# joesound212985/Deepfake-Detection-using-CLIP-Based-SigLIP-2-Vision-Transformers

Hardware: AMD Instinct MI355X
Metric: images/sec (train fwd+bwd) SigLIP-2-so400m@384 bf16 (higher is better)
Workload: dtype bf16; 1 GPU; so400m-patch14-384 encoder+pool-head train fwd+bwd, 384x384, per-GPU batch 128, seeded random weights; global_batch=128, parallelism=dp1

## Files before the change

deepfake-detection-using-clip-based-siglip-2-vision-transformers_amd/csrc/attention.hip:

```cpp
#include <stdlib.h>

#include "common.hip.h"
#include "kernels.h"

namespace sgl {

hipError_t attn_f32_fwd(const float*, const float*, const float*, float*, float*, int, int, int, int, int, int, hipStream_t);
hipError_t attn_f32_bwd(const float*, const float*, const float*, const float*, const float*, const float*, float*,
                        float*, int, int, int, int, int, int, hipStream_t);
hipError_t attn_ref_fwd(const float*, const float*, const float*, float*, float*, int, int, int, int, int, int, hipStream_t);
hipError_t attn_ref_bwd(const float*, const float*, const float*, const float*, const float*, const float*, float*,
                        float*, int, int, int, int, int, int, hipStream_t);

template <int DP>
struct AttnCfg {
  static constexpr int KS = DP / 16;
  static constexpr int DT = (DP + 31) / 32;
  static constexpr int CPR = DP / 8;
  static constexpr int RSTR = DP * 2 + 16;
  static constexpr int TSTR = 192;
  static constexpr int DSTR = 208;
};

__device__ __forceinline__ u32x4 a_ldg(__amdgpu_buffer_rsrc_t r, uint32_t off) {
  return __builtin_amdgcn_raw_buffer_load_b128(r, off, 0, 0);
}
template <typename T>
__device__ __forceinline__ lo_x8<T> as_x8(u32x4 v) { return __builtin_bit_cast(lo_x8<T>, v); }
template <typename T>
__device__ __forceinline__ lo_x8<T> lds_row8(const char* p) { return *reinterpret_cast<const lo_x8<T>*>(p); }
template <typename T>
__device__ __forceinline__ lo_x4<T> lds_tr4(const char* p) { return lds_read_tr16<T>(p); }
template <typename T>
__device__ __forceinline__ lo_x8<T> lds_trfrag(const char* img, int stride, int kk, int dcol0, int lane) {
  const int g = lane >> 4, q = (lane >> 2) & 3, p = lane & 3;
  const char* a = img + (16 * kk + 4 * (g >> 1) + q) * stride + (dcol0 + 16 * (g & 1) + 4 * p) * 2;
  const lo_x4<T> lo = lds_tr4<T>(a);
  const lo_x4<T> hi = lds_tr4<T>(a + 8 * stride);
  return __builtin_shufflevector(lo, hi, 0, 1, 2, 3, 4, 5, 6, 7);
}
template <typename T>
__device__ __forceinline__ lo_x8<T> pack8(const f32x16& s, int base) {
  lo_x8<T> r;
#pragma unroll
  for (int j = 0; j < 8; ++j) r[j] = (T)s[base + j];
  return r;
}
__device__ __forceinline__ float fast_exp2(float x) { return __builtin_amdgcn_exp2f(x); }

__device__ __forceinline__ bool head_block(int nb, int BH, int& bh, int& xb) {
  const int pid = blockIdx.x, xcd = pid & 7, slot = pid >> 3;
  const int hq = slot / nb;
  bh = hq * 8 + xcd;
  xb = slot - hq * nb;
  return bh < BH;
}
static inline dim3 head_grid(int nb, int BH) { return dim3((unsigned)(8 * ((BH + 7) / 8) * nb)); }

struct HeadSrc {
  uint32_t rowbytes, nc, bytes;
  size_t base;
};
__device__ __forceinline__ HeadSrc head_src(int ld, int b, int hd, int H, int N, int dh, int DP) {
  HeadSrc r;
  if (ld > 0) {
    r.rowbytes = (uint32_t)ld * 2u;
    r.nc = (uint32_t)dh / 8u;
    r.bytes = (uint32_t)(((size_t)(N - 1) * ld + dh) * 2);
    r.base = (size_t)b * N * ld + (size_t)hd * dh;
  } else {
    r.rowbytes = (uint32_t)DP * 2u;
    r.nc = (uint32_t)DP / 8u;
    r.bytes = (uint32_t)((size_t)N * DP * 2);
    r.base = ((size_t)b * H + hd) * (size_t)N * DP;
  }
  return r;
}

#define MFMA32(a, b, c) mfma_32x32x16((a), (b), (c))

__device__ __forceinline__ void att_dma16(u32x4 desc, uint32_t lds_addr, uint32_t voff) {
  asm volatile("s_mov_b32 m0, %0\n\ts_nop 0\n\tbuffer_load_dwordx4 %1, %2, 0 offen lds" ::"s"(lds_addr), "v"(voff), "s"(desc)
               : "memory");
}
__device__ __forceinline__ void att_dma4(u32x4 desc, uint32_t lds_addr, uint32_t voff) {
  asm volatile("s_mov_b32 m0, %0\n\ts_nop 0\n\tbuffer_load_dword %1, %2, 0 offen lds" ::"s"(lds_addr), "v"(voff), "s"(desc)
               : "memory");
}
__device__ __forceinline__ u32x4 att_desc(const void* base, uint32_t bytes) {
  const uint64_t q = (uint64_t)base;
  return u32x4{(uint32_t)q, (uint32_t)(q >> 32) & 0xffffu, bytes, 0x00020000u};
}
__device__ __forceinline__ uint32_t att_chunk_off(int cidx, int rows, int SC, int NC, uint32_t rowbytes) {
  const int row = cidx / SC, col = cidx - row * SC;
  return (row < rows && col < NC) ? (uint32_t)row * rowbytes + (uint32_t)col * 16u : SGL_OOB;
}
#define SGL_ATT_WAIT_BARRIER(n)                                   \
  do {                                                            \
    asm volatile("s_waitcnt vmcnt(" #n ") lgkmcnt(0)" ::: "memory"); \
    __builtin_amdgcn_sched_barrier(0);                            \
    __builtin_amdgcn_s_barrier();                                 \
    __builtin_amdgcn_sched_barrier(0);                            \
    asm volatile("" ::: "memory");                                \
  } while (0)

template <typename T, int DP, bool TOK>
__global__ __launch_bounds__(256) __attribute__((amdgpu_waves_per_eu(3, 3))) void attn_fwd_kernel(const T* __restrict__ Q, const T* __restrict__ K,
                                                          const T* __restrict__ V, T* __restrict__ out,
                                                          float* __restrict__ lse, int B, int H, int N, int dh, int ld,
                                                          float c, float scale) {
  using C = AttnCfg<DP>;
  constexpr int KT = 64;
  constexpr int KBYTES = KT * C::RSTR, VBYTES = KT * C::TSTR, STAGE = KBYTES + VBYTES;
  constexpr int SCK = C::RSTR / 16, SCV = C::TSTR / 16;
  constexpr int NIK = KT * SCK / 64, NIV = KT * SCV / 64, NSLOT = NIK + NIV;
  constexpr int NPW = (NSLOT + 3) / 4;
  static_assert(KT * SCK % 64 == 0 && KT * SCV % 64 == 0, "whole DMA instructions per image");
  extern __shared__ __attribute__((aligned(16))) char smem[];
  const int t = threadIdx.x, lane = t & 63;
  const int w = __builtin_amdgcn_readfirstlane(t >> 6);
  int bh, xb;
  if (!head_block((N + 127) / 128, B * H, bh, xb)) return;
  const int b = bh / H, hd = bh - b * H;
  const int q0 = xb * 128 + w * 32;
  HeadSrc src = head_src(TOK ? ld : 0, b, hd, H, N, dh, DP);
  if constexpr (!TOK) {
    src.rowbytes = (uint32_t)DP * 2u;
    src.nc = (uint32_t)DP / 8u;
  }
  const __amdgpu_buffer_rsrc_t rq = make_rsrc(Q + src.base, src.bytes);
  const u32x4 dk_ = att_desc(K + src.base, src.bytes);
  const u32x4 dv_ = att_desc(V + src.base, src.bytes);
  const uint32_t lds0 = (uint32_t)(size_t)((SGL_LDS char*)smem);

  const int qi = lane & 31, hh = lane >> 5;
  lo_x8<T> qf[C::KS];
#pragma unroll
  for (int ks = 0; ks < C::KS; ++ks) {
    const uint32_t ch = (uint32_t)(2 * ks + hh);
    qf[ks] = as_x8<T>(a_ldg(rq, (q0 + qi < N && ch < src.nc) ? (uint32_t)(q0 + qi) * src.rowbytes + ch * 16u : SGL_OOB));
  }

  uint32_t voff[NPW];
#pragma unroll
  for (int j = 0; j < NPW; ++j) {
    const int sl = w + 4 * j;
    voff[j] = (sl < NIK) ? att_chunk_off(sl * 64 + lane, KT, SCK, (int)src.nc, src.rowbytes)
                         : att_chunk_off((sl - NIK) * 64 + lane, KT, SCV, (int)src.nc, src.rowbytes);
  }
  const uint32_t tile_adv = (uint32_t)KT * src.rowbytes;
  auto issue = [&](int stage) {
    const uint32_t sb = lds0 + (uint32_t)(stage * STAGE);
#pragma unroll
    for (int j = 0; j < NPW; ++j) {
      const int sl = w + 4 * j;
      if (sl < NSLOT) att_dma16(sl < NIK ? dk_ : dv_, sb + (uint32_t)sl * 1024u, voff[j]);
      voff[j] += tile_adv;
    }
  };

  float m_run = -INFINITY, l_run = 0.f;
  f32x16 o[C::DT];
#pragma unroll
  for (int dt = 0; dt < C::DT; ++dt)
#pragma unroll
    for (int r = 0; r < 16; ++r) o[dt][r] = 0.f;

  const int ntiles = (N + KT - 1) / KT;
#pragma unroll
  for (int ks = 0; ks < C::KS; ++ks) asm volatile("" ::"v"(qf[ks]));
  asm volatile("s_waitcnt vmcnt(0)" ::: "memory");
  issue(0);
  for (int tile = 0; tile < ntiles; ++tile) {
    const int cur = tile & 1;
    SGL_ATT_WAIT_BARRIER(0);
    if (tile + 1 < ntiles) issue(cur ^ 1);
    const char* kb = smem + cur * STAGE;
    const char* vb = kb + KBYTES;
    f32x16 s0, s1;
#pragma unroll
    for (int r = 0; r < 16; ++r) { s0[r] = 0.f; s1[r] = 0.f; }
#pragma unroll
    for (int ks = 0; ks < C::KS; ++ks) {
      const lo_x8<T> k0 = lds_row8<T>(kb + qi * C::RSTR + (16 * ks + 8 * hh) * 2);
      const lo_x8<T> k1 = lds_row8<T>(kb + (qi + 32) * C::RSTR + (16 * ks + 8 * hh) * 2);
      s0 = MFMA32(k0, qf[ks], s0);
      s1 = MFMA32(k1, qf[ks], s1);
    }
    if (tile == ntiles - 1) {
#pragma unroll
      for (int r = 0; r < 16; ++r) {
        const int key = tile * KT + (r & 3) + 8 * (r >> 2) + 4 * hh;
        if (key >= N) s0[r] = -INFINITY;
        if (key + 32 >= N) s1[r] = -INFINITY;
      }
    }
    float mx = s0[0];
#pragma unroll
    for (int r = 1; r < 16; ++r) mx = fmaxf(mx, s0[r]);
#pragma unroll
    for (int r = 0; r < 16; ++r) mx = fmaxf(mx, s1[r]);
    mx = fmaxf(mx, __shfl_xor(mx, 32, 64));
    const float m_new = fmaxf(m_run, mx);
    const bool grew = __any(m_new > m_run);
    const float alpha = grew ? fast_exp2(c * (m_run - m_new)) : 1.0f;
    const float mc = m_new * c;
    float rs = 0.f;
#pragma unroll
    for (int r = 0; r < 16; ++r) {
      s0[r] = fast_exp2(fmaf(s0[r], c, -mc));
      s1[r] = fast_exp2(fmaf(s1[r], c, -mc));
      rs += s0[r] + s1[r];
    }
    l_run = l_run * alpha + rs;
    m_run = m_new;
    if (grew) {
#pragma unroll
      for (int dt = 0; dt < C::DT; ++dt)
#pragma unroll
        for (int r = 0; r < 16; ++r) o[dt][r] *= alpha;
    }
    lo_x8<T> pb[4];
    pb[0] = pack8<T>(s0, 0);
    pb[1] = pack8<T>(s0, 8);
    pb[2] = pack8<T>(s1, 0);
    pb[3] = pack8<T>(s1, 8);
#pragma unroll
    for (int dt = 0; dt < C::DT; ++dt)
#pragma unroll
      for (int kk = 0; kk < 4; ++kk) o[dt] = MFMA32(lds_trfrag<T>(vb, C::TSTR, kk, dt * 32, lane), pb[kk], o[dt]);
  }
  const float l = l_run + __shfl_xor(l_run, 32, 64);
  const float inv = 1.0f / l;
  const int q = q0 + qi;
  if (q < N) {
    T* orow = out + ((size_t)b * N + q) * ((size_t)H * dh) + hd * dh;
#pragma unroll
    for (int dt = 0; dt < C::DT; ++dt)
#pragma unroll
      for (int g4 = 0; g4 < 4; ++g4) {
        const int d = dt * 32 + 8 * g4 + 4 * hh;
        if (d < dh) {
          lo_x4<T> v4;
#pragma unroll
          for (int r = 0; r < 4; ++r) v4[r] = (T)(o[dt][4 * g4 + r] * inv);
          *reinterpret_cast<lo_x4<T>*>(orow + d) = v4;
        }
      }
    if (hh == 0) lse[(size_t)bh * N + q] = m_run * scale + __logf(l);
  }
}

template <typename T, int DP, bool TOK>
__global__ __launch_bounds__(256, 2) void attn_bwd_kv_kernel(const T* __restrict__ Q, const T* __restrict__ K,
                                                             const T* __restrict__ V, const T* __restrict__ dO,
                                                             const float* __restrict__ aux, T* __restrict__ dqkv,
                                                             int B, int H, int N, int dh, int ld, float c, float scale) {
  using C = AttnCfg<DP>;
  constexpr int QT = 32;
  constexpr int SC = C::DSTR / 16;
  constexpr int NIS = (QT * SC + 63) / 64;
  constexpr int IMG = NIS * 1024;
  constexpr int STAGE = 2 * IMG + QT * 8;
  constexpr int NSLOT = 2 * NIS + 1;
  static_assert(NSLOT <= 16 && NSLOT > 12, "four DMA slots per wave (three for the last wave)");
  extern __shared__ __attribute__((aligned(16))) char smem[];
  const int t = threadIdx.x, lane = t & 63;
  const int w = __builtin_amdgcn_readfirstlane(t >> 6);
  int bh, xb;
  if (!head_block((N + 127) / 128, B * H, bh, xb)) return;
  const int b = bh / H, hd = bh - b * H;
  const int D = H * dh;
  const int key0 = xb * 128 + w * 32;
  HeadSrc src = head_src(TOK ? ld : 0, b, hd, H, N, dh, DP);
  if constexpr (!TOK) {
    src.rowbytes = (uint32_t)DP * 2u;
    src.nc = (uint32_t)DP / 8u;
  }
  const __amdgpu_buffer_rsrc_t rk = make_rsrc(K + src.base, src.bytes);
  const __amdgpu_buffer_rsrc_t rv = make_rsrc(V + src.base, src.bytes);
  const T* dOb = dO + (size_t)b * N * D + hd * dh;
  const u32x4 dq_ = att_desc(Q + src.base, src.bytes);
  const u32x4 ddo = att_desc(dOb, (uint32_t)(((size_t)(N - 1) * D + dh) * 2));
  const u32x4 dax = att_desc(aux + (size_t)bh * N * 2, (uint32_t)((size_t)N * 8));
  const uint32_t lds0 = (uint32_t)(size_t)((SGL_LDS char*)smem);

  const int li = lane & 31, hh = lane >> 5;
  lo_x8<T> kfr[C::KS], vfr[C::KS];
#pragma unroll
  for (int ks = 0; ks < C::KS; ++ks) {
    const uint32_t ch = (uint32_t)(2 * ks + hh);
    const uint32_t off = (key0 + li < N && ch < src.nc) ? (uint32_t)(key0 + li) * src.rowbytes + ch * 16u : SGL_OOB;
    kfr[ks] = as_x8<T>(a_ldg(rk, off));
    vfr[ks] = as_x8<T>(a_ldg(rv, off));
  }

  uint32_t voff[4], vadv[4];
  u32x4 dsc[3];
#pragma unroll
  for (int j = 0; j < 4; ++j) {
    const int sl = w + 4 * j;
    if (sl < NIS) {
      voff[j] = att_chunk_off(sl * 64 + lane, QT, SC, (int)src.nc, src.rowbytes);
      vadv[j] = (uint32_t)QT * src.rowbytes;
    } else if (sl < 2 * NIS) {
      voff[j] = att_chunk_off((sl - NIS) * 64 + lane, QT, SC, dh / 8, (uint32_t)D * 2u);
      vadv[j] = (uint32_t)(QT * D * 2);
    } else {
      voff[j] = (uint32_t)lane * 4u;
      vadv[j] = (uint32_t)(QT * 8);
    }
    if (j < 3) dsc[j] = (sl < NIS) ? dq_ : ddo;
  }
  auto issue1 = [&](int j, int stage) {
    const uint32_t sb = lds0 + (uint32_t)(stage * STAGE) + (uint32_t)w * 1024u;
    if (j < 3) {
      att_dma16(dsc[j], sb + (uint32_t)j * 4096u, voff[j]);
    } else {
      if (w < 2) att_dma16(ddo, sb + 3u * 4096u, voff[3]);
      else if (w == 2) att_dma4(dax, lds0 + (uint32_t)(stage * STAGE + 2 * IMG), voff[3]);
    }
    voff[j] += vadv[j];
  };
  auto issue = [&](int stage) {
#pragma unroll
    for (int j = 0; j < 4; ++j) issue1(j, stage);
  };

  f32x16 dk[C::DT], dv[C::DT];
#pragma unroll
  for (int dt = 0; dt < C::DT; ++dt)
#pragma unroll
    for (int r = 0; r < 16; ++r) { dk[dt][r] = 0.f; dv[dt][r] = 0.f; }

  const int ntiles = (N + QT - 1) / QT;
#pragma unroll
  for (int ks = 0; ks < C::KS; ++ks) asm volatile("" ::"v"(kfr[ks]), "v"(vfr[ks]));
  asm volatile("s_waitcnt vmcnt(0)" ::: "memory");
  issue(0);
  issue(1);
  int st = 0;
  for (int qt = 0; qt < ntiles; ++qt) {
    if (w == 3) SGL_ATT_WAIT_BARRIER(3); else SGL_ATT_WAIT_BARRIER(4);
    const int st_next = (st == 0) ? 2 : st - 1;
    const char* qimg = smem + st * STAGE;
    const char* dimg = qimg + IMG;
    const float* ld = reinterpret_cast<const float*>(qimg + 2 * IMG);
    st = (st == 2) ? 0 : st + 1;
    f32x16 S, dP;
#pragma unroll
    for (int r = 0; r < 16; ++r) { S[r] = 0.f; dP[r] = 0.f; }
    lo_x8<T> qa[C::KS], da[C::KS];
#pragma unroll
    for (int ks = 0; ks < C::KS; ++ks) {
      qa[ks] = lds_row8<T>(qimg + li * C::DSTR + (16 * ks + 8 * hh) * 2);
      da[ks] = lds_row8<T>(dimg + li * C::DSTR + (16 * ks + 8 * hh) * 2);
    }
#pragma unroll
    for (int ks = 0; ks < C::KS; ++ks) {
      S = MFMA32(qa[ks], kfr[ks], S);
      dP = MFMA32(da[ks], vfr[ks], dP);
    }
    if constexpr (C::KS == 5) {
      __builtin_amdgcn_sched_group_barrier(0x100, 4, 0);
#pragma unroll
      for (int i = 0; i < 6; ++i) {
        __builtin_amdgcn_sched_group_barrier(0x008, 1, 0);
        __builtin_amdgcn_sched_group_barrier(0x100, 1, 0);
      }
      __builtin_amdgcn_sched_group_barrier(0x008, 4, 0);
    }
    __builtin_amdgcn_sched_barrier(0);
    constexpr int NF = 2 * 2 * C::DT;
    lo_x8<T> fr[NF];
    auto frag = [&](int i) {
      const int which = i & 1, kk = (i >> 1) & 1, dt = i >> 2;
      return lds_trfrag<T>(which ? qimg : dimg, C::DSTR, kk, dt * 32, lane);
    };
    constexpr int PRE = NF < 2 ? NF : 2;
#pragma unroll
    for (int i = 0; i < PRE; ++i) fr[i] = frag(i);
    __builtin_amdgcn_sched_barrier(0);
#pragma unroll
    for (int g4 = 0; g4 < 4; ++g4) {
      const f32x4 A0 = *reinterpret_cast<const f32x4*>(ld + 2 * (8 * g4 + 4 * hh));
      const f32x4 A1 = *reinterpret_cast<const f32x4*>(ld + 2 * (8 * g4 + 4 * hh) + 4);
      const float L4[4] = {A0[0], A0[2], A1[0], A1[2]};
      const float D4[4] = {A0[1], A0[3], A1[1], A1[3]};
#pragma unroll
      for (int r3 = 0; r3 < 4; ++r3) {
        const int r = 4 * g4 + r3;
        const float p = fast_exp2(fmaf(S[r], c, L4[r3]));
        S[r] = p;
        dP[r] = p * fmaf(dP[r], scale, D4[r3]);
      }
    }
    lo_x8<T> pb[2], dsb[2];
    pb[0] = pack8<T>(S, 0);
    pb[1] = pack8<T>(S, 8);
    dsb[0] = pack8<T>(dP, 0);
    dsb[1] = pack8<T>(dP, 8);
    __builtin_amdgcn_sched_barrier(0);
#pragma unroll
    for (int i = 0; i < NF; ++i) {
      if (i + PRE < NF) fr[i + PRE] = frag(i + PRE);
      const int which = i & 1, kk = (i >> 1) & 1, dt = i >> 2;
      if (which) dk[dt] = MFMA32(fr[i], dsb[kk], dk[dt]);
      else dv[dt] = MFMA32(fr[i], pb[kk], dv[dt]);
      if (i % 3 == 1) issue1(i / 3, st_next);
      __builtin_amdgcn_sched_barrier(0);
    }
#pragma unroll
    for (int j = (NF + 1) / 3; j < 4; ++j) issue1(j, st_next);
  }
  asm volatile("s_waitcnt vmcnt(0)" ::: "memory");
  const int key = key0 + li;
  if (key < N) {
    T* krow = dqkv + ((size_t)b * N + key) * (3 * (size_t)D) + D + hd * dh;
    T* vrow = krow + D;
#pragma unroll
    for (int dt = 0; dt < C::DT; ++dt)
#pragma unroll
      for (int g4 = 0; g4 < 4; ++g4) {
        const int d = dt * 32 + 8 * g4 + 4 * hh;
        if (d < dh) {
          lo_x4<T> a, g;
#pragma unroll
          for (int r = 0; r < 4; ++r) {
            a[r] = (T)dk[dt][4 * g4 + r];
            g[r] = (T)dv[dt][4 * g4 + r];
          }
          *reinterpret_cast<lo_x4<T>*>(krow + d) = a;
          *reinterpret_cast<lo_x4<T>*>(vrow + d) = g;
        }
      }
  }
}

template <typename T, int DP, bool TOK>
__global__ __launch_bounds__(256, 2) void attn_bwd_q_kernel(const T* __restrict__ Q, const T* __restrict__ K,
                                                            const T* __restrict__ V, const T* __restrict__ O,
                                                            const T* __restrict__ dO, const float* __restrict__ lse,
                                                            float* __restrict__ aux, T* __restrict__ dqkv,
                                                            int B, int H, int N, int dh, int ld, float c, float scale) {
  using C = AttnCfg<DP>;
  constexpr int KT = 32;
  constexpr int SCK = C::DSTR / 16, SCV = C::RSTR / 16;
  constexpr int NIK = (KT * SCK + 63) / 64, NIV = (KT * SCV + 63) / 64;
  constexpr int KIMG = NIK * 1024, VIMG = NIV * 1024, STAGE = KIMG + VIMG;
  constexpr int NSLOT = NIK + NIV;
  static_assert(NSLOT <= 16, "at most four DMA slots per wave");
  constexpr float LOG2E = 1.4426950408889634f;
  extern __shared__ __attribute__((aligned(16))) char smem[];
  const int t = threadIdx.x, lane = t & 63;
  const int w = __builtin_amdgcn_readfirstlane(t >> 6);
  int bh, xb;
  if (!head_block((N + 127) / 128, B * H, bh, xb)) return;
  const int b = bh / H, hd = bh - b * H;
  const int D = H * dh;
  const int q0 = xb * 128 + w * 32;
  HeadSrc src = head_src(TOK ? ld : 0, b, hd, H, N, dh, DP);
  if constexpr (!TOK) {
    src.rowbytes = (uint32_t)DP * 2u;
    src.nc = (uint32_t)DP / 8u;
  }
  const __amdgpu_buffer_rsrc_t rq = make_rsrc(Q + src.base, src.bytes);
  const T* dOb = dO + (size_t)b * N * D + hd * dh;
  const __amdgpu_buffer_rsrc_t rdo = make_rsrc(dOb, (uint32_t)(((size_t)(N - 1) * D + dh) * 2));
  const u32x4 dk_ = att_desc(K + src.base, src.bytes);
  const u32x4 dv_ = att_desc(V + src.base, src.bytes);
  const uint32_t lds0 = (uint32_t)(size_t)((SGL_LDS char*)smem);

  const int li = lane & 31, hh = lane >> 5;
  const int q = q0 + li;
  lo_x8<T> qf[C::KS], dof[C::KS];
#pragma unroll
  for (int ks = 0; ks < C::KS; ++ks) {
    const int col = 16 * ks + 8 * hh;
    qf[ks] = as_x8<T>(a_ldg(rq, (q < N && (uint32_t)(col >> 3) < src.nc) ? (uint32_t)q * src.rowbytes + (uint32_t)col * 2u
                                                                           : SGL_OOB));
    dof[ks] = as_x8<T>(a_ldg(rdo, (q < N && col < dh) ? (uint32_t)(((size_t)q * D + col) * 2) : SGL_OOB));
  }
  float dl = 0.f;
  {
    const __amdgpu_buffer_rsrc_t ro = make_rsrc(O + (size_t)b * N * D + hd * dh, (uint32_t)(((size_t)(N - 1) * D + dh) * 2));
#pragma unroll
    for (int ks = 0; ks < C::KS; ++ks) {
      const int col = 16 * ks + 8 * hh;
      const lo_x8<T> of = as_x8<T>(a_ldg(ro, (q < N && col < dh) ? (uint32_t)(((size_t)q * D + col) * 2) : SGL_OOB));
#pragma unroll
      for (int j = 0; j < 8; ++j) dl = fmaf((float)of[j], (float)dof[ks][j], dl);
    }
    dl += __shfl_xor(dl, 32, 64);
  }
  const float Lq = (q < N) ? -lse[(size_t)bh * N + q] * LOG2E : -INFINITY;
  const float Dq = (q < N) ? -dl * scale : 0.f;
  if (q < N && hh == 0) *reinterpret_cast<float2*>(aux + 2 * ((size_t)bh * N + q)) = make_float2(Lq, Dq);

  uint32_t voff[4];
  u32x4 dsc[4];
  uint32_t ldst[4];
#pragma unroll
  for (int j = 0; j < 4; ++j) {
    const int sl = w + 4 * j;
    if (sl < NIK) {
      voff[j] = att_chunk_off(sl * 64 + lane, KT, SCK, (int)src.nc, src.rowbytes);
      dsc[j] = dk_;
      ldst[j] = (uint32_t)sl * 1024u;
    } else {
      voff[j] = att_chunk_off((sl - NIK) * 64 + lane, KT, SCV, (int)src.nc, src.rowbytes);
      dsc[j] = dv_;
      ldst[j] = (uint32_t)(KIMG + (sl - NIK) * 1024);
    }
  }
  auto issue1 = [&](int j, int stage) {
    if (w + 4 * j < NSLOT) att_dma16(dsc[j], lds0 + (uint32_t)(stage * STAGE) + ldst[j], voff[j]);
    voff[j] += (uint32_t)KT * src.rowbytes;
  };

  f32x16 dq[C::DT];
#pragma unroll
  for (int dt = 0; dt < C::DT; ++dt)
#pragma unroll
    for (int r = 0; r < 16; ++r) dq[dt][r] = 0.f;

  const int ntiles = (N + KT - 1) / KT;
#pragma unroll
  for (int ks = 0; ks < C::KS; ++ks) asm volatile("" ::"v"(qf[ks]), "v"(dof[ks]));
  asm volatile("" ::"v"(Lq), "v"(Dq));
  asm volatile("s_waitcnt vmcnt(0)" ::: "memory");
#pragma unroll
  for (int j = 0; j < 4; ++j) issue1(j, 0);
#pragma unroll
  for (int j = 0; j < 4; ++j) issue1(j, 1);
  int st = 0;
  for (int kt = 0; kt < ntiles; ++kt) {
    const int nw = (NSLOT - w + 3) / 4;
    if (nw >= 4) SGL_ATT_WAIT_BARRIER(4);
    else if (nw == 3) SGL_ATT_WAIT_BARRIER(3);
    else if (nw == 2) SGL_ATT_WAIT_BARRIER(2);
    else SGL_ATT_WAIT_BARRIER(1);
    const int st_next = (st == 0) ? 2 : st - 1;
    const char* kimg = smem + st * STAGE;
    const char* vimg = kimg + KIMG;
    st = (st == 2) ? 0 : st + 1;
    f32x16 S, dP;
#pragma unroll
    for (int r = 0; r < 16; ++r) { S[r] = 0.f; dP[r] = 0.f; }
    lo_x8<T> ka[C::KS], va[C::KS];
#pragma unroll
    for (int ks = 0; ks < C::KS; ++ks) {
      ka[ks] = lds_row8<T>(kimg + li * C::DSTR + (16 * ks + 8 * hh) * 2);
      va[ks] = lds_row8<T>(vimg + li * C::RSTR + (16 * ks + 8 * hh) * 2);
    }
#pragma unroll
    for (int ks = 0; ks < C::KS; ++ks) {
      S = MFMA32(ka[ks], qf[ks], S);
      dP = MFMA32(va[ks], dof[ks], dP);
    }
    if constexpr (C::KS == 5) {
      __builtin_amdgcn_sched_group_barrier(0x100, 6, 0);
#pragma unroll
      for (int i = 0; i < 4; ++i) {
        __builtin_amdgcn_sched_group_barrier(0x008, 1, 0);
        __builtin_amdgcn_sched_group_barrier(0x100, 1, 0);
      }
      __builtin_amdgcn_sched_group_barrier(0x008, 6, 0);
    }
    __builtin_amdgcn_sched_barrier(0);
    lo_x8<T> kt_frag[C::DT][2];
#pragma unroll
    for (int dt = 0; dt < C::DT; ++dt)
#pragma unroll
      for (int kk = 0; kk < 2; ++kk) kt_frag[dt][kk] = lds_trfrag<T>(kimg, C::DSTR, kk, dt * 32, lane);
    __builtin_amdgcn_sched_barrier(0);
#pragma unroll
    for (int r = 0; r < 16; ++r) {
      const float p = fast_exp2(fmaf(S[r], c, Lq));
      dP[r] = p * fmaf(dP[r], scale, Dq);
    }
    if (kt == ntiles - 1) {
#pragma unroll
      for (int r = 0; r < 16; ++r) {
        const int key = kt * KT + (r & 3) + 8 * (r >> 2) + 4 * hh;
        if (key >= N) dP[r] = 0.f;
      }
    }
    lo_x8<T> dsb[2];
    dsb[0] = pack8<T>(dP, 0);
    dsb[1] = pack8<T>(dP, 8);
#pragma unroll
    for (int i = 0; i < 2 * C::DT; ++i) {
      dq[i >> 1] = MFMA32(kt_frag[i >> 1][i & 1], dsb[i & 1], dq[i >> 1]);
      if (i < 4) issue1(i, st_next);
      __builtin_amdgcn_sched_barrier(0);
    }
#pragma unroll
    for (int j = 2 * C::DT; j < 4; ++j) issue1(j, st_next);
  }
  asm volatile("s_waitcnt vmcnt(0)" ::: "memory");
  if (q < N) {
    T* qrow = dqkv + ((size_t)b * N + q) * (3 * (size_t)D) + hd * dh;
#pragma unroll
    for (int dt = 0; dt < C::DT; ++dt)
#pragma unroll
      for (int g4 = 0; g4 < 4; ++g4) {
        const int d = dt * 32 + 8 * g4 + 4 * hh;
        if (d < dh) {
          lo_x4<T> a;
#pragma unroll
          for (int r = 0; r < 4; ++r) a[r] = (T)dq[dt][4 * g4 + r];
          *reinterpret_cast<lo_x4<T>*>(qrow + d) = a;
        }
      }
  }
}

template <typename T, int DP>
static hipError_t fwd_launch(const T* q, const T* k, const T* v, T* out, float* lse, int B, int H, int N,
                             int dh, int ld, hipStream_t s) {
  using C = AttnCfg<DP>;
  constexpr int smem = 2 * (64 * C::RSTR + 64 * C::TSTR);
  const float scale = 1.0f / sqrtf((float)dh);
  if (ld > 0)
    hipLaunchKernelGGL((attn_fwd_kernel<T, DP, true>), head_grid((N + 127) / 128, B * H), dim3(256), smem, s, q, k, v, out, lse,
                       B, H, N, dh, ld, scale * 1.4426950408889634f, scale);
  else
    hipLaunchKernelGGL((attn_fwd_kernel<T, DP, false>), head_grid((N + 127) / 128, B * H), dim3(256), smem, s, q, k, v, out,
                       lse, B, H, N, dh, 0, scale * 1.4426950408889634f, scale);
  return hipGetLastError();
}

template <typename T, int DP>
static hipError_t bwd_launch(const T* q, const T* k, const T* v, const T* out, const T* dout,
                             const float* lse, T* dqkv, float* delta, int B, int H, int N, int dh, int ld,
                             hipStream_t s) {
  using C = AttnCfg<DP>;
  const float scale = 1.0f / sqrtf((float)dh);
  const float c = scale * 1.4426950408889634f;
  constexpr int smem_kv = 3 * (2 * ((32 * (C::DSTR / 16) + 63) / 64) * 1024 + 32 * 8);
  constexpr int smem_q = 3 * (((32 * (C::DSTR / 16) + 63) / 64) + ((32 * (C::RSTR / 16) + 63) / 64)) * 1024;
  const dim3 grid = head_grid((N + 127) / 128, B * H), block(256);
  if (ld > 0)
    hipLaunchKernelGGL((attn_bwd_q_kernel<T, DP, true>), grid, block, smem_q, s, q, k, v, out, dout, lse, delta, dqkv, B, H, N,
                       dh, ld, c, scale);
  else
    hipLaunchKernelGGL((attn_bwd_q_kernel<T, DP, false>), grid, block, smem_q, s, q, k, v, out, dout, lse, delta, dqkv, B, H, N,
                       dh, 0, c, scale);
  hipError_t e = hipGetLastError();
  if (e != hipSuccess) return e;
  if (ld > 0)
    hipLaunchKernelGGL((attn_bwd_kv_kernel<T, DP, true>), grid, block, smem_kv, s, q, k, v, dout, delta, dqkv, B, H, N, dh, ld, c,
                       scale);
  else
    hipLaunchKernelGGL((attn_bwd_kv_kernel<T, DP, false>), grid, block, smem_kv, s, q, k, v, dout, delta, dqkv, B, H, N, dh, 0,
                       c, scale);
  return hipGetLastError();
}

static bool attn_shape_ok(int N, int dh, int DP, int H, int ld) {
  if (dh % 8 || DP != ((dh + 15) / 16) * 16) return false;
  if (DP != 16 && DP != 32 && DP != 48 && DP != 64 && DP != 80 && DP != 96) return false;
  if (ld < 0 || (ld > 0 && (ld % 8 || ld < H * dh))) return false;
  if ((size_t)N * (ld > 0 ? ld : DP) * 2 >= (1ull << 31)) return false;
  if ((size_t)N * H * dh * 2 >= (1ull << 31)) return false;
  return true;
}

hipError_t attn_fwd(const void* q, const void* k, const void* v, int dtype, void* out, float* lse, int B, int H, int N,
                    int dh, int DP, int ld, hipStream_t s) {
  if (B * H == 0 || N == 0) return hipSuccess;
  if (dtype == DT_F32)
    return attn_ref_fwd((const float*)q, (const float*)k, (const float*)v, (float*)out, lse, B, H, N, dh, DP, ld, s);
  if (dtype == DT_F32_MFMA)
    return attn_f32_fwd((const float*)q, (const float*)k, (const float*)v, (float*)out, lse, B, H, N, dh, DP, ld, s);
  if (!attn_shape_ok(N, dh, DP, H, ld)) return hipErrorInvalidValue;
  if ((((uintptr_t)q) | ((uintptr_t)k) | ((uintptr_t)v)) & 15) return hipErrorInvalidValue;
#define SGL_F(T, DPV) \
  case DPV: return fwd_launch<T, DPV>((const T*)q, (const T*)k, (const T*)v, (T*)out, lse, B, H, N, dh, ld, s);
  if (dtype == DT_F16) {
    switch (DP) {
      SGL_F(f16, 16) SGL_F(f16, 32) SGL_F(f16, 48) SGL_F(f16, 64) SGL_F(f16, 80) SGL_F(f16, 96)
    }
    return hipErrorInvalidValue;
  }
  switch (DP) {
    SGL_F(bf16, 16) SGL_F(bf16, 32) SGL_F(bf16, 48) SGL_F(bf16, 64) SGL_F(bf16, 80) SGL_F(bf16, 96)
  }
#undef SGL_F
  return hipErrorInvalidValue;
}

hipError_t attn_bwd(const void* q, const void* k, const void* v, const void* out, const void* dout, const float* lse,
                    int dtype, void* dqkv, float* delta, float* , int B, int H, int N, int dh, int DP,
                    int ld, hipStream_t s) {
  if (B * H == 0 || N == 0) return hipSuccess;
  if (dtype == DT_F32)
    return attn_ref_bwd((const float*)q, (const float*)k, (const float*)v, (const float*)out, (const float*)dout, lse,
                        (float*)dqkv, delta, B, H, N, dh, DP, ld, s);
  if (dtype == DT_F32_MFMA)
    return attn_f32_bwd((const float*)q, (const float*)k, (const float*)v, (const float*)out, (const float*)dout, lse,
                        (float*)dqkv, delta, B, H, N, dh, DP, ld, s);
  if (!attn_shape_ok(N, dh, DP, H, ld)) return hipErrorInvalidValue;
  if ((((uintptr_t)q) | ((uintptr_t)k) | ((uintptr_t)v)) & 15) return hipErrorInvalidValue;
#define SGL_B(T, DPV)                                                                                  \
  case DPV:                                                                                            \
    return bwd_launch<T, DPV>((const T*)q, (const T*)k, (const T*)v, (const T*)out, (const T*)dout, lse, \
                              (T*)dqkv, delta, B, H, N, dh, ld, s);
  if (dtype == DT_F16) {
    switch (DP) {
      SGL_B(f16, 16) SGL_B(f16, 32) SGL_B(f16, 48) SGL_B(f16, 64) SGL_B(f16, 80) SGL_B(f16, 96)
    }
    return hipErrorInvalidValue;
  }
  switch (DP) {
    SGL_B(bf16, 16) SGL_B(bf16, 32) SGL_B(bf16, 48) SGL_B(bf16, 64) SGL_B(bf16, 80) SGL_B(bf16, 96)
  }
#undef SGL_B
  return hipErrorInvalidValue;
}

}
```

Measured before the change: 439.5 images/sec.

## Use rotated swizzled LDS images in attention backward with precomputed lane bases

Replaces the padded 208-byte-stride LDS tiles for Q/dO/K in both backward kernels with a dense 192-byte rotated-chunk layout. Compile-time checks assert that row and transposed reads are bank-conflict-free. Per-lane LDS base addresses are computed once and pinned, and the 3-stage loop is unrolled so stage offsets become immediates, cutting address arithmetic. The smaller image drops one DMA slot per tile and shrinks LDS, in exchange for a more complex addressing scheme and larger unrolled code.

Result: no change. 440.6 images/sec (median of 3 runs) (+0.2%).

```diff
diff --git a/deepfake-detection-using-clip-based-siglip-2-vision-transformers_amd/csrc/attention.hip b/deepfake-detection-using-clip-based-siglip-2-vision-transformers_amd/csrc/attention.hip
--- a/deepfake-detection-using-clip-based-siglip-2-vision-transformers_amd/csrc/attention.hip
+++ b/deepfake-detection-using-clip-based-siglip-2-vision-transformers_amd/csrc/attention.hip
@@ -19,7 +19,6 @@
   static constexpr int CPR = DP / 8;
   static constexpr int RSTR = DP * 2 + 16;
   static constexpr int TSTR = 192;
-  static constexpr int DSTR = 208;
 };
 
 __device__ __forceinline__ u32x4 a_ldg(__amdgpu_buffer_rsrc_t r, uint32_t off) {
@@ -95,6 +94,127 @@
   const int row = cidx / SC, col = cidx - row * SC;
   return (row < rows && col < NC) ? (uint32_t)row * rowbytes + (uint32_t)col * 16u : SGL_OOB;
 }
+
+namespace att_img {
+constexpr int ROWS = 32, NCH = 12, ROWB = NCH * 16, BYTES = ROWS * ROWB, NDMA = BYTES / 1024;
+static_assert(BYTES % 1024 == 0, "whole DMA instructions per image");
+__host__ __device__ constexpr int slot_of(int row, int chunk) { return (chunk + (row >> 2)) % NCH; }
+__host__ __device__ constexpr int chunk_of(int row, int slot) { return (slot + NCH - (row >> 2)) % NCH; }
+__host__ __device__ constexpr int off(int row, int colb) { return row * ROWB + 16 * slot_of(row, colb >> 4) + (colb & 15); }
+
+__host__ __device__ constexpr int row_off(int lane, int ks) { return off(lane & 31, 32 * ks + 16 * (lane >> 5)); }
+
+__host__ __device__ constexpr int tr_row(int lane) { return 4 * (lane >> 5) + ((lane >> 2) & 3); }
+__host__ __device__ constexpr int tr_colb(int lane) { return 32 * ((lane >> 4) & 1) + 8 * (lane & 3); }
+__host__ __device__ constexpr int tr_off(int lane, int kk, int dt, int half) {
+  return off(16 * kk + 8 * half + tr_row(lane), 64 * dt + tr_colb(lane));
+}
+__host__ __device__ constexpr int tr_B(int kk, int dt, int half) { return (4 * (dt + kk) + 2 * half) % NCH; }
+__host__ __device__ constexpr int tr_sel(int kk, int dt, int half) { return tr_B(kk, dt, half) < 8 ? 0 : tr_B(kk, dt, half) == 8 ? 1 : 2; }
+__host__ __device__ constexpr int tr_base(int lane, int sel) {
+  return sel == 0 ? tr_off(lane, 0, 0, 0) : sel == 1 ? tr_off(lane, 0, 2, 0) : tr_off(lane, 0, 2, 1) - 8 * ROWB;
+}
+__host__ __device__ constexpr bool tr_uses(int DT, int sel) {
+  for (int kk = 0; kk < 2; ++kk)
+    for (int dt = 0; dt < DT; ++dt)
+      for (int half = 0; half < 2; ++half)
+        if (tr_sel(kk, dt, half) == sel) return true;
+  return false;
+}
+__host__ __device__ constexpr int tr_imm(int kk, int dt, int half) {
+  return (16 * kk + 8 * half) * ROWB + (tr_B(kk, dt, half) < 8 ? 16 * tr_B(kk, dt, half) : 0);
+}
+
+constexpr int b128_group(int lane) {
+  const int l = lane & 31;
+  return ((l < 4 || (l >= 12 && l < 16) || (l >= 20 && l < 28)) ? 0 : 1) + 2 * (lane >> 5);
+}
+constexpr int b64_group(int lane) { return lane >> 5; }
+template <typename Addr, typename Group>
+constexpr int lds_cycles(Addr addr, Group group, int ngroups, int dwords) {
+  int total = 0;
+  for (int g = 0; g < ngroups; ++g) {
+    int seen[64 * 4] = {}, nseen = 0, load[64] = {}, worst = 0;
+    for (int lane = 0; lane < 64; ++lane) {
+      if (group(lane) != g) continue;
+      for (int d = 0; d < dwords; ++d) {
+        const int dw = addr(lane) / 4 + d;
+        bool dup = false;
+        for (int i = 0; i < nseen; ++i) dup = dup || seen[i] == dw;
+        if (dup) continue;
+        seen[nseen++] = dw;
+        if (++load[dw % 64] > worst) worst = load[dw % 64];
+      }
+    }
+    total += worst;
+  }
+  return total;
+}
+struct RowAddr { int ks; constexpr int operator()(int lane) const { return row_off(lane, ks); } };
+struct TrAddr { int kk, dt, half; constexpr int operator()(int lane) const { return tr_base(lane, tr_sel(kk, dt, half)) + tr_imm(kk, dt, half); } };
+struct G128 { constexpr int operator()(int lane) const { return b128_group(lane); } };
+struct G64 { constexpr int operator()(int lane) const { return b64_group(lane); } };
+constexpr bool check_inverse() {
+  for (int r = 0; r < ROWS; ++r)
+    for (int c = 0; c < NCH; ++c)
+      if (chunk_of(r, slot_of(r, c)) != c || off(r, 16 * c) < 0 || off(r, 16 * c) + 16 > BYTES) return false;
+  return true;
+}
+constexpr bool check_tr_bases() {
+  for (int lane = 0; lane < 64; ++lane)
+    for (int kk = 0; kk < 2; ++kk)
+      for (int dt = 0; dt < 3; ++dt)
+        for (int half = 0; half < 2; ++half)
+          if (TrAddr{kk, dt, half}(lane) != tr_off(lane, kk, dt, half)) return false;
+  return true;
+}
+constexpr int row_read_cycles() {
+  int n = 0;
+  for (int ks = 0; ks < 6; ++ks) n += lds_cycles(RowAddr{ks}, G128{}, 4, 4);
+  return n;
+}
+constexpr int tr_read_cycles() {
+  int n = 0;
+  for (int kk = 0; kk < 2; ++kk)
+    for (int dt = 0; dt < 3; ++dt)
+      for (int half = 0; half < 2; ++half) n += lds_cycles(TrAddr{kk, dt, half}, G64{}, 2, 2);
+  return n;
+}
+static_assert(check_inverse(), "slot_of / chunk_of are inverse permutations inside the image");
+static_assert(check_tr_bases(), "three per-lane bases + immediates reproduce every transposed read address");
+static_assert(row_read_cycles() == 6 * 4, "row reads (ds_read_b128, 4 x 16 lanes) of the rotated image are conflict-free");
+static_assert(tr_read_cycles() == 12 * 2, "transposed reads (ds_read_b64_tr_b16, 2 x 32 lanes) are conflict-free");
+}
+
+__device__ __forceinline__ uint32_t att_img_chunk_off(int cidx, int NC, uint32_t rowbytes) {
+  const int row = cidx / att_img::NCH, col = att_img::chunk_of(row, cidx - row * att_img::NCH);
+  return (row < att_img::ROWS && col < NC) ? (uint32_t)row * rowbytes + (uint32_t)col * 16u : SGL_OOB;
+}
+__device__ __forceinline__ uint32_t att_lds_pin(uint32_t a) {
+  asm volatile("" : "+v"(a));
+  return a;
+}
+__device__ __forceinline__ const char* att_lds_ptr(uint32_t a) { return (const char*)(SGL_LDS const char*)(size_t)a; }
+struct AttImgLane {
+  uint32_t row[6];
+  uint32_t tr[3];
+};
+template <int KS, int DT>
+__device__ __forceinline__ AttImgLane att_img_lane(uint32_t img0, int lane) {
+  AttImgLane a;
+#pragma unroll
+  for (int ks = 0; ks < 6; ++ks) a.row[ks] = ks < KS ? att_lds_pin(img0 + (uint32_t)att_img::row_off(lane, ks)) : 0u;
+#pragma unroll
+  for (int s = 0; s < 3; ++s) a.tr[s] = att_img::tr_uses(DT, s) ? att_lds_pin(img0 + (uint32_t)att_img::tr_base(lane, s)) : 0u;
+  return a;
+}
+template <typename T>
+__device__ __forceinline__ lo_x8<T> att_img_trfrag(const AttImgLane& a, int d, int kk, int dt) {
+  const lo_x4<T> lo = lds_tr4<T>(att_lds_ptr(a.tr[att_img::tr_sel(kk, dt, 0)] + (uint32_t)(d + att_img::tr_imm(kk, dt, 0))));
+  const lo_x4<T> hi = lds_tr4<T>(att_lds_ptr(a.tr[att_img::tr_sel(kk, dt, 1)] + (uint32_t)(d + att_img::tr_imm(kk, dt, 1))));
+  return __builtin_shufflevector(lo, hi, 0, 1, 2, 3, 4, 5, 6, 7);
+}
+
 #define SGL_ATT_WAIT_BARRIER(n)                                   \
   do {                                                            \
     asm volatile("s_waitcnt vmcnt(" #n ") lgkmcnt(0)" ::: "memory"); \
@@ -258,12 +378,12 @@
                                                              int B, int H, int N, int dh, int ld, float c, float scale) {
   using C = AttnCfg<DP>;
   constexpr int QT = 32;
-  constexpr int SC = C::DSTR / 16;
-  constexpr int NIS = (QT * SC + 63) / 64;
-  constexpr int IMG = NIS * 1024;
+  constexpr int NIS = att_img::NDMA;
+  constexpr int IMG = att_img::BYTES;
   constexpr int STAGE = 2 * IMG + QT * 8;
   constexpr int NSLOT = 2 * NIS + 1;
-  static_assert(NSLOT <= 16 && NSLOT > 12, "four DMA slots per wave (three for the last wave)");
+  static_assert(QT == att_img::ROWS, "one image per tile");
+  static_assert(NSLOT <= 16 && NSLOT > 12 && NSLOT == 13, "three image slots per wave, a fourth (the pairs) on wave 0");
   extern __shared__ __attribute__((aligned(16))) char smem[];
   const int t = threadIdx.x, lane = t & 63;
   const int w = __builtin_amdgcn_readfirstlane(t >> 6);
@@ -301,10 +421,10 @@
   for (int j = 0; j < 4; ++j) {
     const int sl = w + 4 * j;
     if (sl < NIS) {
-      voff[j] = att_chunk_off(sl * 64 + lane, QT, SC, (int)src.nc, src.rowbytes);
+      voff[j] = att_img_chunk_off(sl * 64 + lane, (int)src.nc, src.rowbytes);
       vadv[j] = (uint32_t)QT * src.rowbytes;
     } else if (sl < 2 * NIS) {
-      voff[j] = att_chunk_off((sl - NIS) * 64 + lane, QT, SC, dh / 8, (uint32_t)D * 2u);
+      voff[j] = att_img_chunk_off((sl - NIS) * 64 + lane, dh / 8, (uint32_t)D * 2u);
       vadv[j] = (uint32_t)(QT * D * 2);
     } else {
       voff[j] = (uint32_t)lane * 4u;
@@ -317,8 +437,7 @@
     if (j < 3) {
       att_dma16(dsc[j], sb + (uint32_t)j * 4096u, voff[j]);
     } else {
-      if (w < 2) att_dma16(ddo, sb + 3u * 4096u, voff[3]);
-      else if (w == 2) att_dma4(dax, lds0 + (uint32_t)(stage * STAGE + 2 * IMG), voff[3]);
+      if (w == 0) att_dma4(dax, lds0 + (uint32_t)(stage * STAGE + 2 * IMG), voff[3]);
     }
     voff[j] += vadv[j];
   };
@@ -339,22 +458,23 @@
   asm volatile("s_waitcnt vmcnt(0)" ::: "memory");
   issue(0);
   issue(1);
-  int st = 0;
-  for (int qt = 0; qt < ntiles; ++qt) {
-    if (w == 3) SGL_ATT_WAIT_BARRIER(3); else SGL_ATT_WAIT_BARRIER(4);
+  const AttImgLane ia = att_img_lane<C::KS, C::DT>(lds0, lane);
+  const uint32_t ldp = att_lds_pin(lds0 + (uint32_t)(2 * IMG + 8 * (4 * hh)));
+  for (int qt0 = 0; qt0 < ntiles; qt0 += 3) {
+#pragma unroll
+  for (int st = 0; st < 3; ++st) {
+    if (qt0 + st >= ntiles) break;
+    if (w == 0) SGL_ATT_WAIT_BARRIER(4); else SGL_ATT_WAIT_BARRIER(3);
     const int st_next = (st == 0) ? 2 : st - 1;
-    const char* qimg = smem + st * STAGE;
-    const char* dimg = qimg + IMG;
-    const float* ld = reinterpret_cast<const float*>(qimg + 2 * IMG);
-    st = (st == 2) ? 0 : st + 1;
+    const int qimg = st * STAGE, dimg = qimg + IMG;
     f32x16 S, dP;
 #pragma unroll
     for (int r = 0; r < 16; ++r) { S[r] = 0.f; dP[r] = 0.f; }
     lo_x8<T> qa[C::KS], da[C::KS];
 #pragma unroll
     for (int ks = 0; ks < C::KS; ++ks) {
-      qa[ks] = lds_row8<T>(qimg + li * C::DSTR + (16 * ks + 8 * hh) * 2);
-      da[ks] = lds_row8<T>(dimg + li * C::DSTR + (16 * ks + 8 * hh) * 2);
+      qa[ks] = lds_row8<T>(att_lds_ptr(ia.row[ks] + (uint32_t)qimg));
+      da[ks] = lds_row8<T>(att_lds_ptr(ia.row[ks] + (uint32_t)dimg));
     }
 #pragma unroll
     for (int ks = 0; ks < C::KS; ++ks) {
@@ -375,7 +495,7 @@
     lo_x8<T> fr[NF];
     auto frag = [&](int i) {
       const int which = i & 1, kk = (i >> 1) & 1, dt = i >> 2;
-      return lds_trfrag<T>(which ? qimg : dimg, C::DSTR, kk, dt * 32, lane);
+      return att_img_trfrag<T>(ia, which ? qimg : dimg, kk, dt);
     };
     constexpr int PRE = NF < 2 ? NF : 2;
 #pragma unroll
@@ -383,8 +503,8 @@
     __builtin_amdgcn_sched_barrier(0);
 #pragma unroll
     for (int g4 = 0; g4 < 4; ++g4) {
-      const f32x4 A0 = *reinterpret_cast<const f32x4*>(ld + 2 * (8 * g4 + 4 * hh));
-      const f32x4 A1 = *reinterpret_cast<const f32x4*>(ld + 2 * (8 * g4 + 4 * hh) + 4);
+      const f32x4 A0 = *reinterpret_cast<const f32x4*>(att_lds_ptr(ldp + (uint32_t)(qimg + 64 * g4)));
+      const f32x4 A1 = *reinterpret_cast<const f32x4*>(att_lds_ptr(ldp + (uint32_t)(qimg + 64 * g4 + 16)));
       const float L4[4] = {A0[0], A0[2], A1[0], A1[2]};
       const float D4[4] = {A0[1], A0[3], A1[1], A1[3]};
 #pragma unroll
@@ -412,6 +532,7 @@
     }
 #pragma unroll
     for (int j = (NF + 1) / 3; j < 4; ++j) issue1(j, st_next);
+  }
   }
   asm volatile("s_waitcnt vmcnt(0)" ::: "memory");
   const int key = key0 + li;
@@ -445,10 +566,11 @@
                                                             int B, int H, int N, int dh, int ld, float c, float scale) {
   using C = AttnCfg<DP>;
   constexpr int KT = 32;
-  constexpr int SCK = C::DSTR / 16, SCV = C::RSTR / 16;
-  constexpr int NIK = (KT * SCK + 63) / 64, NIV = (KT * SCV + 63) / 64;
-  constexpr int KIMG = NIK * 1024, VIMG = NIV * 1024, STAGE = KIMG + VIMG;
+  constexpr int SCV = C::RSTR / 16;
+  constexpr int NIK = att_img::NDMA, NIV = (KT * SCV + 63) / 64;
+  constexpr int KIMG = att_img::BYTES, VIMG = NIV * 1024, STAGE = KIMG + VIMG;
   constexpr int NSLOT = NIK + NIV;
+  static_assert(KT == att_img::ROWS, "one image per tile");
   static_assert(NSLOT <= 16, "at most four DMA slots per wave");
   constexpr float LOG2E = 1.4426950408889634f;
   extern __shared__ __attribute__((aligned(16))) char smem[];
@@ -504,7 +626,7 @@
   for (int j = 0; j < 4; ++j) {
     const int sl = w + 4 * j;
     if (sl < NIK) {
-      voff[j] = att_chunk_off(sl * 64 + lane, KT, SCK, (int)src.nc, src.rowbytes);
+      voff[j] = att_img_chunk_off(sl * 64 + lane, (int)src.nc, src.rowbytes);
       dsc[j] = dk_;
       ldst[j] = (uint32_t)sl * 1024u;
     } else {
@@ -533,25 +655,28 @@
   for (int j = 0; j < 4; ++j) issue1(j, 0);
 #pragma unroll
   for (int j = 0; j < 4; ++j) issue1(j, 1);
-  int st = 0;
-  for (int kt = 0; kt < ntiles; ++kt) {
+  const AttImgLane ia = att_img_lane<C::KS, C::DT>(lds0, lane);
+  const uint32_t vrow = att_lds_pin(lds0 + (uint32_t)(KIMG + li * C::RSTR + 16 * hh));
+  for (int kt0 = 0; kt0 < ntiles; kt0 += 3) {
+#pragma unroll
+  for (int st = 0; st < 3; ++st) {
+    const int kt = kt0 + st;
+    if (kt >= ntiles) break;
     const int nw = (NSLOT - w + 3) / 4;
     if (nw >= 4) SGL_ATT_WAIT_BARRIER(4);
     else if (nw == 3) SGL_ATT_WAIT_BARRIER(3);
     else if (nw == 2) SGL_ATT_WAIT_BARRIER(2);
     else SGL_ATT_WAIT_BARRIER(1);
     const int st_next = (st == 0) ? 2 : st - 1;
-    const char* kimg = smem + st * STAGE;
-    const char* vimg = kimg + KIMG;
-    st = (st == 2) ? 0 : st + 1;
+    const int kimg = st * STAGE;
     f32x16 S, dP;
 #pragma unroll
     for (int r = 0; r < 16; ++r) { S[r] = 0.f; dP[r] = 0.f; }
     lo_x8<T> ka[C::KS], va[C::KS];
 #pragma unroll
     for (int ks = 0; ks < C::KS; ++ks) {
-      ka[ks] = lds_row8<T>(kimg + li * C::DSTR + (16 * ks + 8 * hh) * 2);
-      va[ks] = lds_row8<T>(vimg + li * C::RSTR + (16 * ks + 8 * hh) * 2);
+      ka[ks] = lds_row8<T>(att_lds_ptr(ia.row[ks] + (uint32_t)kimg));
+      va[ks] = lds_row8<T>(att_lds_ptr(vrow + (uint32_t)(kimg + 32 * ks)));
     }
 #pragma unroll
     for (int ks = 0; ks < C::KS; ++ks) {
@@ -572,7 +697,7 @@
 #pragma unroll
     for (int dt = 0; dt < C::DT; ++dt)
 #pragma unroll
-      for (int kk = 0; kk < 2; ++kk) kt_frag[dt][kk] = lds_trfrag<T>(kimg, C::DSTR, kk, dt * 32, lane);
+      for (int kk = 0; kk < 2; ++kk) kt_frag[dt][kk] = att_img_trfrag<T>(ia, kimg, kk, dt);
     __builtin_amdgcn_sched_barrier(0);
 #pragma unroll
     for (int r = 0; r < 16; ++r) {
@@ -597,6 +722,7 @@
     }
 #pragma unroll
     for (int j = 2 * C::DT; j < 4; ++j) issue1(j, st_next);
+  }
   }
   asm volatile("s_waitcnt vmcnt(0)" ::: "memory");
   if (q < N) {
@@ -638,8 +764,8 @@
   using C = AttnCfg<DP>;
   const float scale = 1.0f / sqrtf((float)dh);
   const float c = scale * 1.4426950408889634f;
-  constexpr int smem_kv = 3 * (2 * ((32 * (C::DSTR / 16) + 63) / 64) * 1024 + 32 * 8);
-  constexpr int smem_q = 3 * (((32 * (C::DSTR / 16) + 63) / 64) + ((32 * (C::RSTR / 16) + 63) / 64)) * 1024;
+  constexpr int smem_kv = 3 * (2 * att_img::BYTES + 32 * 8);
+  constexpr int smem_q = 3 * (att_img::BYTES + ((32 * (C::RSTR / 16) + 63) / 64) * 1024);
   const dim3 grid = head_grid((N + 127) / 128, B * H), block(256);
   if (ld > 0)
     hipLaunchKernelGGL((attn_bwd_q_kernel<T, DP, true>), grid, block, smem_q, s, q, k, v, out, dout, lse, delta, dqkv, B, H, N,
```
